# Yukun-Huang/DreamWaltz-G

Measured on AMD Instinct MI355X. Metric: SDS steps/sec @512^2, 100k Gaussians, SD1.5+ControlNet; raster Mpix/s vs HBM roofline, higher is better.
Workload: dtype f32x

## Files before the change

### dreamwaltz-g_amd/csrc/gemm.hip

```cpp
#include "dwg_common.h"
#include "dwg_prof_internal.h"
#include "../../include/dwg_gemm.h"
#include <cstdlib>
#include <type_traits>

#if defined(DWG_GEMM_X_TU)
#include "dwg_xfmt.h"
typedef _Float16 HT;
#define DWG_DTYPE_HALF DWG_DTYPE_F32X
#define DWG_MFMA16(a, b, c) __builtin_amdgcn_mfma_f32_32x32x16_f16(a, b, c, 0, 0, 0)
#define DWG_HALF_NAME "f32x"
#elif defined(DWG_GEMM_F16_TU)
typedef _Float16 HT;
#define DWG_DTYPE_HALF DWG_DTYPE_F16
#define DWG_MFMA16(a, b, c) __builtin_amdgcn_mfma_f32_32x32x16_f16(a, b, c, 0, 0, 0)
#define DWG_HALF_NAME "f16"
#else
typedef __bf16 HT;
#define DWG_DTYPE_HALF DWG_DTYPE_BF16
#define DWG_MFMA16(a, b, c) __builtin_amdgcn_mfma_f32_32x32x16_bf16(a, b, c, 0, 0, 0)
#define DWG_HALF_NAME "bf16"
#endif

namespace {

typedef __attribute__((ext_vector_type(8))) HT bf16x8;
typedef __attribute__((ext_vector_type(16))) float f32x16;

struct ConvP {
    int enabled, Cin, Hin, Win, Hout, Wout, KH, KW, stride, pad_t, pad_l, dil;
    int up;
    int cin1;
    const void* A2;
};

struct GemmP {
    const void* A; const void* B; void* C; const void* bias; const void* residual;
    int M, N, K;
    long long sam, sak, sbn, sbk, ldc, ldr;
    int nb2;
    long long bA1, bA2, bB1, bB2, bC1, bC2, bR1, bR2;
    int act; float alpha;
    int out_bf16, res_bf16, bias_per_row, splitk, accumulate;
    float* ws;
    int bias_row_div;
    long long bias_ld;
    ConvP conv;
};

__device__ __forceinline__ float bf2f(HT x) { return (float)x; }
// ... 249 lines not shown
            float4 r = *reinterpret_cast<const float4*>(reinterpret_cast<const float*>(p.residual) + ri);
            v[0] += r.x; v[1] += r.y; v[2] += r.z; v[3] += r.w;
        }
    }
    const long long ci = coff + (long long)row * p.ldc + col;
    if (p.out_bf16) {
        st_half4(p.C, ci, v);
    } else {
        float4* dst = reinterpret_cast<float4*>(reinterpret_cast<float*>(p.C) + ci);
        float4 o = make_float4(v[0], v[1], v[2], v[3]);
        if (p.accumulate) { float4 c = *dst; o.x += c.x; o.y += c.y; o.z += c.z; o.w += c.w; }
        *dst = o;
    }
}

template <int BN, int BM = 128> struct EpiLds {
    static constexpr int LDC = BN + 4;
    static constexpr int passes(size_t lds_bytes) {
        return lds_bytes >= (size_t)BM * LDC * 4 ? 1 : (lds_bytes >= (size_t)(BM / 2) * LDC * 4 ? 2 : 4);
    }
    static constexpr size_t bytes(int npass) { return (size_t)(BM / npass) * LDC * 4; }
};

template <int BN, int NPASS, int TM, int TN, bool LIGHT, int BM = 128, int NT = 256, typename RowFn>
__device__ __forceinline__ void tile_epilogue_lds(const GemmP& p, f32x16 (&acc)[TM][TN], float* sC, int n0, int wm, int wn, int lane, int tid,
                                                  int ks_id, long long coff, long long roff, RowFn row_of) {
    constexpr int LDC = EpiLds<BN, BM>::LDC, C4 = BN / 4, PR = BM / NPASS;
    constexpr int BPP = BM / 32 / NPASS;
    static_assert(NT % C4 == 0 && (C4 & (C4 - 1)) == 0, "a thread keeps one column group");
    const bool vec_ok = epilogue_vec_ok(p, coff, roff);
    const int lrow = lane & 31, lhalf = (lane >> 5) * 4;
    const bool geglu = p.act == 6;
    const float* bias = reinterpret_cast<const float*>(p.bias);
    const bool fast = vec_ok && !geglu && !p.accumulate && !p.bias_per_row && (p.splitk <= 1 || p.ws) &&
                      (!bias || p.bias_row_div > 0 || ((uintptr_t)bias & 15) == 0) &&
                      (!bias || p.bias_row_div <= 0 || (((uintptr_t)bias & 15) == 0 && (p.bias_ld & 3) == 0)) &&
                      (p.splitk <= 1 || ((uintptr_t)p.ws & 15) == 0);
#pragma unroll 1
    for (int q = 0; q < NPASS; q++) {
        __syncthreads();
#pragma unroll
        for (int i = 0; i < TM; i++) {
            const int rb = wm * TM + i;
            if (NPASS > 1 && rb / BPP != q) continue;
            float* dst = sC + ((NPASS > 1 ? rb % BPP : rb) * 32 + lrow) * LDC + wn * 64 + lhalf;
#pragma unroll
            for (int j = 0; j < TN; j++)
#pragma unroll
                for (int r4 = 0; r4 < 4; r4++)
                    *reinterpret_cast<float4*>(dst + j * 32 + 8 * r4) =
                        make_float4(acc[i][j][4 * r4], acc[i][j][4 * r4 + 1], acc[i][j][4 * r4 + 2], acc[i][j][4 * r4 + 3]);
        }
        __syncthreads();
        if (geglu) {
            constexpr int G = C4 / 2, RSTEP = NT / G;
            const int o4 = tid & (G - 1), rl0 = tid / G;
            const int b = o4 >> 3, w = (o4 & 7) * 4;
            const int colp = n0 + b * 64 + w;
            if (colp + 35 < p.N) {
                float bh[4] = {0.f, 0.f, 0.f, 0.f}, bg[4] = {0.f, 0.f, 0.f, 0.f};
                if (bias) {
#pragma unroll
                    for (int e = 0; e < 4; e++) { bh[e] = bias[colp + e]; bg[e] = bias[colp + 32 + e]; }
                }
                const bool vec_store = ((p.ldc | coff) & 3) == 0 && ((uintptr_t)p.C & 7) == 0;
#pragma unroll 2
                for (int rl = rl0; rl < PR; rl += RSTEP) {
                    const int row = row_of(q * PR + rl);
                    if (row < 0) continue;
                    const float4 h = *reinterpret_cast<const float4*>(sC + rl * LDC + b * 64 + w);
                    const float4 g = *reinterpret_cast<const float4*>(sC + rl * LDC + b * 64 + 32 + w);
                    const float hv[4] = {h.x, h.y, h.z, h.w}, gv[4] = {g.x, g.y, g.z, g.w};
                    float v[4];
#pragma unroll
// ... 344 lines not shown
    }
    __device__ __forceinline__ void issue(unsigned char* lds_tile, const ConvP& cv) {
        const int wave = __builtin_amdgcn_readfirstlane(threadIdx.x >> 6);
        const unsigned char* zero = g_zero16;
        const bool second = CAT && ci >= cv.cin1;
        const int cs = CAT ? (second ? cv.Cin - cv.cin1 : cv.cin1) : cv.Cin;
        const long long uoff = (((long long)ky * cv.Win + kx) * cs + (second ? ci - cv.cin1 : ci)) * 2;
        const unsigned int bit = kcur < kend ? (1u << tap) : 0u;
#pragma unroll
        for (int j = 0; j < NJ; j++) {
            const unsigned char* src = (mask[j] & bit) ? ((CAT && second) ? pb2[j] : pb[j]) + uoff : zero;
            unsigned char* dst = lds_tile + ((wave * NJ + j) * 8) * 128;
            __builtin_amdgcn_global_load_lds((const __attribute__((address_space(1))) void*)src,
                                             (__attribute__((address_space(3))) void*)dst, 16, 0, 0);
        }
    }
};

template <int N>
__device__ __forceinline__ void wait_vmcnt() {
    __builtin_amdgcn_s_waitcnt((N & 15) | ((N >> 4) << 14) | (7 << 4) | (15 << 8));
}

template <int BM, int AKIND, int NW = 4> struct ALoaderOf { typedef GldsLoader<BM, false, NW> type; };
template <int BM, int NW> struct ALoaderOf<BM, 1, NW> { typedef GldsLoader<BM, true, NW> type; };
template <int BM, int NW> struct ALoaderOf<BM, 2, NW> { typedef GldsConvFast<BM, NW, false> type; };
template <int BM, int NW> struct ALoaderOf<BM, 3, NW> { typedef GldsConvFast<BM, NW, true> type; };

template <int BM, int BN> struct GldsGeom {
    static constexpr int WN = BN / 64, WM = (BM == 128 && BN == 64) ? 4 : BM / 64, NW = WM * WN, NT = NW * 64, TM = BM / WM / 32, TN = 2;
};

template <int BM, int BN, int AKIND, int S>
__device__ __forceinline__ void gemm_glds_body(const GemmP& p) {
    typedef GldsGeom<BM, BN> Geo;
    constexpr int WN = Geo::WN, WM = Geo::WM, NW = Geo::NW, NT = Geo::NT, TM = Geo::TM, TN = Geo::TN;
    constexpr int ABYTES = BM * 128, BBYTES = BN * 128, STAGE = ABYTES + BBYTES;
    extern __shared__ __attribute__((aligned(16))) unsigned char smem_raw[];
    const int tid = threadIdx.x, lane = tid & 63, wave = tid >> 6;
    const int wm = wave / WN, wn = wave % WN;
    const int gm = (p.M + BM - 1) / BM, ntn = (p.N + BN - 1) / BN;
    const int nwg = gridDim.x;
    int id = blockIdx.x;
    {
        const int q = nwg / 8, r = nwg % 8, xcd = id % 8, loc = id / 8;
        id = (xcd < r ? xcd * (q + 1) : r * (q + 1) + (xcd - r) * q) + loc;
    }
    const int tile = id % (gm * ntn), ks_id = id / (gm * ntn);
    const int m0 = (tile / ntn) * BM, n0 = (tile % ntn) * BN;
    const int z = blockIdx.z, z1 = z / p.nb2, z2 = z - z1 * p.nb2;
    const HT* A = reinterpret_cast<const HT*>(p.A) + z1 * p.bA1 + z2 * p.bA2;
    const HT* B = reinterpret_cast<const HT*>(p.B) + z1 * p.bB1 + z2 * p.bB2;
    int kbeg = 0, kend = p.K;
    if (p.splitk > 1) {
        int per = ((p.K + p.splitk - 1) / p.splitk + 63) / 64 * 64;
        kbeg = ks_id * per; kend = min(p.K, kbeg + per);
    }
    f32x16 acc[TM][TN];
#pragma unroll
    for (int i = 0; i < TM; i++)
#pragma unroll
        for (int j = 0; j < TN; j++)
#pragma unroll
            for (int r = 0; r < 16; r++) acc[i][j][r] = 0.f;
#ifdef DWG_GEMM_X_TU
    f32x16 acx[TM][TN];
#pragma unroll
    for (int i = 0; i < TM; i++)
#pragma unroll
        for (int j = 0; j < TN; j++)
#pragma unroll
            for (int r = 0; r < 16; r++) acx[i][j][r] = 0.f;
#endif
    typename ALoaderOf<BM, AKIND, NW>::type la;
    GldsLoader<BN, false, NW> lb;
    la.init(A, p.sam, p.M, m0, kbeg, kend, p.conv);
    lb.init(B, p.sbn, p.N, n0, kbeg, kend, p.conv);
    const int nk = kend > kbeg ? (kend - kbeg + 63) / 64 : 0;
    constexpr int LPT = (BM + BN) * 128 / (NT * 16);
#pragma unroll
    for (int s = 0; s < S - 1; s++) {
        la.issue(smem_raw + s * STAGE, p.conv); lb.issue(smem_raw + s * STAGE + ABYTES, p.conv);
        la.advance(p.conv); lb.advance(p.conv);
    }
    const int frow = lane & 31, fx = (lane >> 1) & 7, fh = lane >> 5;
#ifdef DWG_GEMM_X_TU
    constexpr int KS = 2;
    struct Frag { bf16x8 ah[TM], al[TM], bh[TN], bl[TN]; };
#else
    constexpr int KS = 4;
    struct Frag { bf16x8 af[TM], bf[TN]; };
#endif
    auto load_frags = [&](int stage, int ks, Frag& f) {
        const unsigned char* ta = smem_raw + stage * STAGE + (wm * TM * 32 + frow) * 128;
        const unsigned char* tb = smem_raw + stage * STAGE + ABYTES + (wn * 64 + frow) * 128;
#ifdef DWG_GEMM_X_TU
        const int offh = (((ks * 4 + fh * 2) ^ fx) << 4), offl = (((ks * 4 + fh * 2 + 1) ^ fx) << 4);
#pragma unroll
        for (int i = 0; i < TM; i++) {
            f.ah[i] = *reinterpret_cast<const bf16x8*>(ta + i * 32 * 128 + offh);
            f.al[i] = *reinterpret_cast<const bf16x8*>(ta + i * 32 * 128 + offl);
        }
#pragma unroll
        for (int j = 0; j < TN; j++) {
            f.bh[j] = *reinterpret_cast<const bf16x8*>(tb + j * 32 * 128 + offh);
            f.bl[j] = *reinterpret_cast<const bf16x8*>(tb + j * 32 * 128 + offl);
        }
#else
        const int off = (((ks * 2 + fh) ^ fx) << 4);
#pragma unroll
        for (int i = 0; i < TM; i++) f.af[i] = *reinterpret_cast<const bf16x8*>(ta + i * 32 * 128 + off);
#pragma unroll
        for (int j = 0; j < TN; j++) f.bf[j] = *reinterpret_cast<const bf16x8*>(tb + j * 32 * 128 + off);
#endif
    };
    auto mma = [&](const Frag& f) {
#ifdef DWG_GEMM_X_TU
#pragma unroll
        for (int i = 0; i < TM; i++)
#pragma unroll
            for (int j = 0; j < TN; j++) acc[i][j] = DWG_MFMA16(f.bh[j], f.ah[i], acc[i][j]);
#pragma unroll
        for (int i = 0; i < TM; i++)
#pragma unroll
            for (int j = 0; j < TN; j++) acx[i][j] = DWG_MFMA16(f.bl[j], f.ah[i], acx[i][j]);
#pragma unroll
        for (int i = 0; i < TM; i++)
#pragma unroll
            for (int j = 0; j < TN; j++) acx[i][j] = DWG_MFMA16(f.bh[j], f.al[i], acx[i][j]);
#else
#pragma unroll
        for (int i = 0; i < TM; i++)
#pragma unroll
            for (int j = 0; j < TN; j++) acc[i][j] = DWG_MFMA16(f.bf[j], f.af[i], acc[i][j]);
#endif
    };
    auto wait_tile_and_lds = [&]() {
        constexpr int N = (S - 2) * LPT;
        __builtin_amdgcn_s_waitcnt((N & 15) | ((N >> 4) << 14) | (7 << 4) | (0 << 8));
    };
    Frag F[2];
    int cur = 0, nxt = S - 1;
    if (nk > 0) {
        wait_vmcnt<(S - 2) * LPT>();
        __builtin_amdgcn_s_barrier();
        load_frags(0, 0, F[0]);
        __builtin_amdgcn_s_waitcnt(0xC07F);
    }
#ifdef DWG_GEMM_X_TU
    constexpr int MPS = 3 * TM * TN;
#else
    constexpr int MPS = TM * TN;
#endif
    for (int kt = 0; kt < nk; kt++) {
        const int cnext = cur + 1 == S ? 0 : cur + 1;
#pragma unroll
        for (int ks = 0; ks < KS; ks++) {
            if (ks + 1 < KS) {
                load_frags(cur, ks + 1, F[(ks + 1) & 1]);
            } else {
                wait_tile_and_lds();
                __builtin_amdgcn_s_barrier();
                load_frags(cnext, 0, F[0]);
            }
            __builtin_amdgcn_sched_barrier(0);
            if (ks == 0) {
                la.issue(smem_raw + nxt * STAGE, p.conv); lb.issue(smem_raw + nxt * STAGE + ABYTES, p.conv);
                la.advance(p.conv); lb.advance(p.conv);
            }
            mma(F[ks & 1]);
            if (ks == 0) {
#pragma unroll
                for (int m = 0; m < MPS; m++) {
                    __builtin_amdgcn_sched_group_barrier(0x008, 1, 0);
                    __builtin_amdgcn_sched_group_barrier(0x006, (LPT * 10 + MPS - 1) / MPS, 0);
                    __builtin_amdgcn_sched_group_barrier(0x020, (LPT + MPS - 1) / MPS, 0);
                }
            }
            __builtin_amdgcn_sched_barrier(0);
        }
        __builtin_amdgcn_s_waitcnt(0xC07F);
        cur = cnext; nxt = nxt + 1 == S ? 0 : nxt + 1;
    }
    wait_vmcnt<0>();
#ifdef DWG_GEMM_X_TU
#pragma unroll
    for (int i = 0; i < TM; i++)
#pragma unroll
        for (int j = 0; j < TN; j++)
#pragma unroll
            for (int r = 0; r < 16; r++) acc[i][j][r] = fmaf(acx[i][j][r], DWG_X_LO_INV, acc[i][j][r]);
#endif
    constexpr int NPASS = EpiLds<BN, BM>::passes((size_t)S * STAGE);
    static_assert((size_t)S * STAGE >= EpiLds<BN, BM>::bytes(NPASS), "epilogue staging fits in the operand stages");
    tile_epilogue_lds<BN, NPASS, TM, TN, false, BM, NT>(p, acc, reinterpret_cast<float*>(smem_raw), n0, wm, wn, lane, tid, ks_id, z1 * p.bC1 + z2 * p.bC2,
                                         z1 * p.bR1 + z2 * p.bR2, [&](int rl) { const int r = m0 + rl; return r < p.M ? r : -1; });
}

template <int BN, int AKIND, int S>
__global__ __launch_bounds__(256, 2) void k_gemm_glds(GemmP p) {
    gemm_glds_body<128, BN, AKIND, S>(p);
}

template <int BM, int BN, int AKIND, int S>
__global__ __launch_bounds__(512, 2) void k_gemm_glds8(GemmP p) {
    static_assert(GldsGeom<BM, BN>::NT == 512, "eight waves");
    gemm_glds_body<BM, BN, AKIND, S>(p);
}

static double gemm_flops(const GemmP& p, int batch) {
    double f = 2.0 * p.M * p.N * p.K * batch;
#ifdef DWG_GEMM_X_TU
    f *= 0.5;
#endif
    if (p.conv.enabled && p.conv.dil > 1) f /= (double)(p.conv.dil * p.conv.dil);
    return f;
}

template <int BN, int AKIND>
static void launch_glds(const GemmP& p, int batch, hipStream_t stream, const char* name) {
    constexpr int S = (BN == 64 && AKIND != 1) ? 3 : 2;
    size_t lds = (size_t)S * (128 + BN) * 128;
    static bool attr_set = false;
// ... 5 lines not shown
    static const char* const sym[2][4] = {{"k_gemm_glds<64, 0, 3>", "k_gemm_glds<64, 1, 2>", "k_gemm_glds<64, 2, 3>", "k_gemm_glds<64, 3, 3>"},
                                          {"k_gemm_glds<128, 0, 2>", "k_gemm_glds<128, 1, 2>", "k_gemm_glds<128, 2, 2>", "k_gemm_glds<128, 3, 2>"}};
    DWG_LAUNCH_W(name, sym[BN == 128][AKIND], gemm_flops(p, batch), (k_gemm_glds<BN, AKIND, S>), grid, dim3(256), lds, stream, p);
    launch_splitk_epilogue(p, stream);
}

template <int BM, int BN, int AKIND>
static void launch_glds8(const GemmP& p, int batch, hipStream_t stream, const char* name) {
    constexpr int S = 3;
    const size_t lds = (size_t)S * (BM + BN) * 128;
    static bool attr_set = false;
    if (!attr_set) {
        hipFuncSetAttribute(reinterpret_cast<const void*>(&k_gemm_glds8<BM, BN, AKIND, S>), hipFuncAttributeMaxDynamicSharedMemorySize, (int)lds);
        attr_set = true;
    }
    dim3 grid(((p.M + BM - 1) / BM) * ((p.N + BN - 1) / BN) * (p.splitk > 1 ? p.splitk : 1), 1, batch);
    static const char* const sym[2][4] = {
        {"k_gemm_glds8<256, 128, 0, 3>", "k_gemm_glds8<256, 128, 1, 3>", "k_gemm_glds8<256, 128, 2, 3>", "k_gemm_glds8<256, 128, 3, 3>"},
        {"k_gemm_glds8<128, 256, 0, 3>", "k_gemm_glds8<128, 256, 1, 3>", "k_gemm_glds8<128, 256, 2, 3>", "k_gemm_glds8<128, 256, 3, 3>"}};
    DWG_LAUNCH_W(name, sym[BN == 256][AKIND], gemm_flops(p, batch), (k_gemm_glds8<BM, BN, AKIND, S>), grid, dim3(512), lds, stream, p);
    launch_splitk_epilogue(p, stream);
}

template <bool V> struct BoolC { static constexpr bool value = V; };
template <int BN, int NW> struct Patch2Geom {
    static constexpr int PH = NW == 8 ? 16 : 8, PW = 16, HP = PH + 2, WP = PW + 2, NPIX = HP * WP, BM = PH * PW;
    static constexpr int NPI = (NPIX + 7) / 8;
    static constexpr int PPW = (NPI + NW - 1) / NW;
    static constexpr int WN = BN / 64, WM = NW / WN, TM = BM / WM / 32, TN = 2, NT = NW * 64;
    static constexpr int NJW = BN / (8 * NW);
    static constexpr int PBYTES = NPI * 8 * 128, BBYTES = BN * 128;
};

template <int BN, bool SPLIT, int NW, int NBS>
__global__ __launch_bounds__(NW * 64, 2) void k_conv3x3_patch2(GemmP p) {
    typedef Patch2Geom<BN, NW> G;
    constexpr int PH = G::PH, PW = G::PW, WP = G::WP, NPIX = G::NPIX, NPI = G::NPI, PPW = G::PPW;
    constexpr int WN = G::WN, WM = G::WM, TM = G::TM, TN = G::TN, NT = G::NT, NJW = G::NJW, BM = G::BM;
    constexpr int PBYTES = G::PBYTES, BBYTES = G::BBYTES;
    static_assert(NJW >= 1 && (NJW % 2 == 0 || NJW == 1), "row-block parity");
    extern __shared__ __attribute__((aligned(16))) unsigned char smem_raw[];
    unsigned char* sP = smem_raw;
    unsigned char* sB = smem_raw + 2 * PBYTES;
    const ConvP& cv = p.conv;
    const int tid = threadIdx.x, lane = tid & 63, wave = tid >> 6;
    const int wv = __builtin_amdgcn_readfirstlane(wave);
    const int wm = wave / WN, wn = wave % WN;
// ... 24 lines not shown
            const int py = pi / WP, px = pi - py * WP;
            const int iy = y0 - 1 + py, ix = x0 - 1 + px;
            const bool ok = valid && pi < NPIX && iy >= 0 && iy < cv.Hin && ix >= 0 && ix < cv.Win;
            const HT* src = ok ? X + ((long long)iy * cv.Win + ix) * cv.Cin + (lg0 ^ ((inst & 1) << 2)) * 8 + cc * 64 : zero;
            __builtin_amdgcn_global_load_lds((const __attribute__((address_space(1))) void*)src,
                                             (__attribute__((address_space(3))) void*)(dst + inst * 8 * 128), 16, 0, 0);
        }
    };
    const HT* wrow[NJW];
#pragma unroll
    for (int j = 0; j < NJW; j++) {
        const int r = n0 + (wv * NJW + j) * 8 + sub;
        wrow[j] = r < p.N ? Wt + (long long)r * p.sbn + (lg0 ^ (((wv * NJW + j) & 1) << 2)) * 8 : nullptr;
    }
    auto issue_w = [&](int cc, int tap, bool valid, unsigned char* dst) {
        const long long kofs = (long long)tap * cv.Cin + cc * 64;
#pragma unroll
        for (int j = 0; j < NJW; j++) {
            const HT* src = (valid && wrow[j]) ? wrow[j] + kofs : zero;
            __builtin_amdgcn_global_load_lds((const __attribute__((address_space(1))) void*)src,
                                             (__attribute__((address_space(3))) void*)(dst + (wv * NJW + j) * 8 * 128), 16, 0, 0);
        }
    };
    f32x16 acc[TM][TN];
#pragma unroll
    for (int i = 0; i < TM; i++)
#pragma unroll
        for (int j = 0; j < TN; j++)
#pragma unroll
            for (int r = 0; r < 16; r++) acc[i][j][r] = 0.f;
#ifdef DWG_GEMM_X_TU
    f32x16 acx[TM][TN];
#pragma unroll
    for (int i = 0; i < TM; i++)
#pragma unroll
        for (int j = 0; j < TN; j++)
#pragma unroll
            for (int r = 0; r < 16; r++) acx[i][j][r] = 0.f;
    constexpr int KS = 2, MPS = 3 * TM * TN;
    struct Frag { bf16x8 ah[TM], al[TM], bh[TN], bl[TN]; };
#else
    constexpr int KS = 4, MPS = TM * TN;
    struct Frag { bf16x8 af[TM], bf[TN]; };
#endif
    int pbase[TM];
#pragma unroll
    for (int i = 0; i < TM; i++) {
        const int r = (wm * TM + i) * 32 + (lane & 31);
        pbase[i] = (r / PW) * WP + (r % PW);
    }
    int cc0 = 0, ncc = cv.Cin / 64;
    if constexpr (SPLIT) {
        const int per = (ncc + p.splitk - 1) / p.splitk;
        cc0 = ks_id * per; ncc = min(ncc, cc0 + per);
    }
    const int frow = lane & 31, fx = (lane >> 1) & 7, fh = lane >> 5;
    const int nsteps = max(0, ncc - cc0) * 9;
    auto load_frags = [&](const unsigned char* pa, int toff, const unsigned char* tbs, int ks, Frag& f) {
        const unsigned char* tb = tbs + (wn * 64 + frow) * 128;
#ifdef DWG_GEMM_X_TU
        const int cl = ks * 4 + fh * 2;
#pragma unroll
        for (int i = 0; i < TM; i++) {
            const int pi = pbase[i] + toff, sw = (pi >> 1) & 7;
            f.ah[i] = *reinterpret_cast<const bf16x8*>(pa + pi * 128 + ((cl ^ sw) << 4));
            f.al[i] = *reinterpret_cast<const bf16x8*>(pa + pi * 128 + (((cl + 1) ^ sw) << 4));
        }
#pragma unroll
        for (int j = 0; j < TN; j++) {
            f.bh[j] = *reinterpret_cast<const bf16x8*>(tb + j * 32 * 128 + ((cl ^ fx) << 4));
            f.bl[j] = *reinterpret_cast<const bf16x8*>(tb + j * 32 * 128 + (((cl + 1) ^ fx) << 4));
        }
#else
        const int cl = ks * 2 + fh;
#pragma unroll
        for (int i = 0; i < TM; i++) {
            const int pi = pbase[i] + toff;
            f.af[i] = *reinterpret_cast<const bf16x8*>(pa + pi * 128 + ((cl ^ ((pi >> 1) & 7)) << 4));
        }
#pragma unroll
        for (int j = 0; j < TN; j++) f.bf[j] = *reinterpret_cast<const bf16x8*>(tb + j * 32 * 128 + ((cl ^ fx) << 4));
#endif
    };
    auto mma = [&](const Frag& f) {
#ifdef DWG_GEMM_X_TU
#pragma unroll
        for (int i = 0; i < TM; i++)
#pragma unroll
            for (int j = 0; j < TN; j++) acc[i][j] = DWG_MFMA16(f.bh[j], f.ah[i], acc[i][j]);
#pragma unroll
        for (int i = 0; i < TM; i++)
#pragma unroll
            for (int j = 0; j < TN; j++) acx[i][j] = DWG_MFMA16(f.bl[j], f.ah[i], acx[i][j]);
#pragma unroll
        for (int i = 0; i < TM; i++)
#pragma unroll
            for (int j = 0; j < TN; j++) acx[i][j] = DWG_MFMA16(f.bh[j], f.al[i], acx[i][j]);
#else
#pragma unroll
        for (int i = 0; i < TM; i++)
#pragma unroll
            for (int j = 0; j < TN; j++) acc[i][j] = DWG_MFMA16(f.bf[j], f.af[i], acc[i][j]);
#endif
    };
    issue_patch(cc0, nsteps > 0, sP + (cc0 & 1) * PBYTES);
#pragma unroll
    for (int g = 0; g < NBS - 1; g++) issue_w(cc0 + g / 9, g % 9, g < nsteps, sB + g * BBYTES);
    Frag F[2];
    if (nsteps > 0) {
        wait_vmcnt<(NBS - 2) * NJW>();
        __builtin_amdgcn_s_barrier();
        load_frags(sP + (cc0 & 1) * PBYTES, 0, sB, 0, F[0]);
        __builtin_amdgcn_s_waitcnt(0xC07F);
    }
    int bst = 0;
    auto step = [&](auto is_tap0, int tap, int cc, const unsigned char* pa, const unsigned char* pan) {
        constexpr bool TAP0 = decltype(is_tap0)::value;
        const int ty = tap >= 6 ? 2 : (tap >= 3 ? 1 : 0);
        const int toff = ty * WP + (tap - 3 * ty);
        const int bnext = bst + 1 == NBS ? 0 : bst + 1;
        const int bfill = bst == 0 ? NBS - 1 : bst - 1;
        const unsigned char* tb = sB + bst * BBYTES;
#pragma unroll
        for (int ks = 0; ks < KS; ks++) {
            if (ks + 1 < KS) {
                load_frags(pa, toff, tb, ks + 1, F[(ks + 1) & 1]);
// ... 11 lines not shown
                load_frags(tap == 8 ? pan : pa, nty * WP + (ntap - 3 * nty), sB + bnext * BBYTES, 0, F[0]);
            }
            __builtin_amdgcn_sched_barrier(0);
            if (ks == 0) {
                const int ft = tap + NBS - 1, fcc = cc + (ft >= 9 ? 1 : 0), ftap = ft >= 9 ? ft - 9 : ft;
                issue_w(fcc, ftap, fcc < ncc, sB + bfill * BBYTES);
                if (TAP0) issue_patch(cc + 1, cc + 1 < ncc, const_cast<unsigned char*>(pan));
            }
            mma(F[ks & 1]);
            if (ks == 0) {
                constexpr int NL = NJW + (TAP0 ? PPW : 0);
#pragma unroll
                for (int m = 0; m < MPS; m++) {
                    __builtin_amdgcn_sched_group_barrier(0x008, 1, 0);
                    __builtin_amdgcn_sched_group_barrier(0x006, (NL * 8 + MPS - 1) / MPS, 0);
                    __builtin_amdgcn_sched_group_barrier(0x020, (NL + MPS - 1) / MPS, 0);
                }
            }
            __builtin_amdgcn_sched_barrier(0);
        }
        __builtin_amdgcn_s_waitcnt(0xC07F);
        bst = bnext;
    };
    for (int cc = cc0; cc < ncc; cc++) {
        const unsigned char* pa = sP + (cc & 1) * PBYTES;
        const unsigned char* pan = sP + ((cc + 1) & 1) * PBYTES;
        step(BoolC<true>{}, 0, cc, pa, pan);
#pragma unroll 1
        for (int tap = 1; tap < 9; tap++) step(BoolC<false>{}, tap, cc, pa, pan);
    }
    wait_vmcnt<0>();
    __builtin_amdgcn_s_barrier();
#ifdef DWG_GEMM_X_TU
#pragma unroll
    for (int i = 0; i < TM; i++)
#pragma unroll
        for (int j = 0; j < TN; j++)
#pragma unroll
            for (int r = 0; r < 16; r++) acc[i][j][r] = fmaf(acx[i][j][r], DWG_X_LO_INV, acc[i][j][r]);
#endif
    constexpr int NPASS = EpiLds<BN, BM>::passes((size_t)2 * PBYTES + NBS * BBYTES);
    static_assert((size_t)2 * PBYTES + NBS * BBYTES >= EpiLds<BN, BM>::bytes(NPASS), "epilogue staging fits in the patch / weight buffers");
    tile_epilogue_lds<BN, NPASS, TM, TN, !SPLIT, BM, NT>(p, acc, reinterpret_cast<float*>(smem_raw), n0, wm, wn, lane, tid, ks_id, 0, 0, [&](int rr) {
        const int y = y0 + rr / PW, x = x0 + rr % PW;
        return (y < cv.Hout && x < cv.Wout) ? (img * cv.Hout + y) * cv.Wout + x : -1;
    });
}

template <int BN, int NW, int NBS>
static void launch_conv3x3_patch2(const GemmP& p, hipStream_t stream, const char* name) {
    typedef Patch2Geom<BN, NW> G;
    const size_t lds = (size_t)2 * G::PBYTES + (size_t)NBS * G::BBYTES;
    const ConvP& cv = p.conv;
    const int nimg = p.M / (cv.Hout * cv.Wout);
    const int gm = nimg * ((cv.Hout + G::PH - 1) / G::PH) * ((cv.Wout + G::PW - 1) / G::PW);
    dim3 grid(gm * ((p.N + BN - 1) / BN) * (p.splitk > 1 ? p.splitk : 1));
    static bool attr_set = false;
    if (!attr_set) {
        hipFuncSetAttribute(reinterpret_cast<const void*>(&k_conv3x3_patch2<BN, false, NW, NBS>), hipFuncAttributeMaxDynamicSharedMemorySize, (int)lds);
        hipFuncSetAttribute(reinterpret_cast<const void*>(&k_conv3x3_patch2<BN, true, NW, NBS>), hipFuncAttributeMaxDynamicSharedMemorySize, (int)lds);
        attr_set = true;
    }
    static_assert((NW == 8 && BN == 128 && NBS == 4) || (NW == 4 && BN == 64 && NBS == 4) || (NW == 4 && BN == 128 && NBS == 2), "symbol table below");
    const char* sym = NW == 8 ? (p.splitk > 1 && p.ws ? "k_conv3x3_patch2<128, true, 8, 4>" : "k_conv3x3_patch2<128, false, 8, 4>")
                              : (BN == 64 ? (p.splitk > 1 && p.ws ? "k_conv3x3_patch2<64, true, 4, 4>" : "k_conv3x3_patch2<64, false, 4, 4>")
                                          : (p.splitk > 1 && p.ws ? "k_conv3x3_patch2<128, true, 4, 2>" : "k_conv3x3_patch2<128, false, 4, 2>"));
// ... 367 lines not shown
```

Before: 41.35.

## Use 16x16x32 MFMA with permlane-swapped split operands for f32x GEMM and conv

```diff
diff --git a/dreamwaltz-g_amd/csrc/gemm.hip b/dreamwaltz-g_amd/csrc/gemm.hip
--- a/dreamwaltz-g_amd/csrc/gemm.hip
+++ b/dreamwaltz-g_amd/csrc/gemm.hip
@@ -3,22 +3,27 @@
 #include "../../include/dwg_gemm.h"
 #include <cstdlib>
 #include <type_traits>
+#include <utility>
 
 #if defined(DWG_GEMM_X_TU)
 #include "dwg_xfmt.h"
 typedef _Float16 HT;
 #define DWG_DTYPE_HALF DWG_DTYPE_F32X
 #define DWG_MFMA16(a, b, c) __builtin_amdgcn_mfma_f32_32x32x16_f16(a, b, c, 0, 0, 0)
+#define DWG_MFMA32(a, b, c) __builtin_amdgcn_mfma_f32_16x16x32_f16(a, b, c, 0, 0, 0)
+#define DWG_MFMA_K32 1
 #define DWG_HALF_NAME "f32x"
 #elif defined(DWG_GEMM_F16_TU)
 typedef _Float16 HT;
 #define DWG_DTYPE_HALF DWG_DTYPE_F16
 #define DWG_MFMA16(a, b, c) __builtin_amdgcn_mfma_f32_32x32x16_f16(a, b, c, 0, 0, 0)
+#define DWG_MFMA_K32 0
 #define DWG_HALF_NAME "f16"
 #else
 typedef __bf16 HT;
 #define DWG_DTYPE_HALF DWG_DTYPE_BF16
 #define DWG_MFMA16(a, b, c) __builtin_amdgcn_mfma_f32_32x32x16_bf16(a, b, c, 0, 0, 0)
+#define DWG_MFMA_K32 0
 #define DWG_HALF_NAME "bf16"
 #endif
 
@@ -26,6 +31,7 @@
 
 typedef __attribute__((ext_vector_type(8))) HT bf16x8;
 typedef __attribute__((ext_vector_type(16))) float f32x16;
+typedef __attribute__((ext_vector_type(4))) float f32x4;
 
 struct ConvP {
     int enabled, Cin, Hin, Win, Hout, Wout, KH, KW, stride, pad_t, pad_l, dil;
@@ -321,11 +327,12 @@
     static constexpr size_t bytes(int npass) { return (size_t)(BM / npass) * LDC * 4; }
 };
 
-template <int BN, int NPASS, int TM, int TN, bool LIGHT, int BM = 128, int NT = 256, typename RowFn>
-__device__ __forceinline__ void tile_epilogue_lds(const GemmP& p, f32x16 (&acc)[TM][TN], float* sC, int n0, int wm, int wn, int lane, int tid,
+template <int BN, int NPASS, int TM, int TN, bool LIGHT, int BM = 128, int NT = 256, typename ACC, typename RowFn>
+__device__ __forceinline__ void tile_epilogue_lds(const GemmP& p, ACC (&acc)[TM][TN], float* sC, int n0, int wm, int wn, int lane, int tid,
                                                   int ks_id, long long coff, long long roff, RowFn row_of) {
     constexpr int LDC = EpiLds<BN, BM>::LDC, C4 = BN / 4, PR = BM / NPASS;
-    constexpr int BPP = BM / 32 / NPASS;
+    constexpr int TR = sizeof(ACC) == sizeof(f32x16) ? 32 : 16;
+    constexpr int BPP = BM / TR / NPASS;
     static_assert(NT % C4 == 0 && (C4 & (C4 - 1)) == 0, "a thread keeps one column group");
     const bool vec_ok = epilogue_vec_ok(p, coff, roff);
     const int lrow = lane & 31, lhalf = (lane >> 5) * 4;
@@ -342,13 +349,20 @@
         for (int i = 0; i < TM; i++) {
             const int rb = wm * TM + i;
             if (NPASS > 1 && rb / BPP != q) continue;
-            float* dst = sC + ((NPASS > 1 ? rb % BPP : rb) * 32 + lrow) * LDC + wn * 64 + lhalf;
-#pragma unroll
-            for (int j = 0; j < TN; j++)
-#pragma unroll
-                for (int r4 = 0; r4 < 4; r4++)
-                    *reinterpret_cast<float4*>(dst + j * 32 + 8 * r4) =
-                        make_float4(acc[i][j][4 * r4], acc[i][j][4 * r4 + 1], acc[i][j][4 * r4 + 2], acc[i][j][4 * r4 + 3]);
+            if constexpr (TR == 32) {
+                float* dst = sC + ((NPASS > 1 ? rb % BPP : rb) * 32 + lrow) * LDC + wn * 64 + lhalf;
+#pragma unroll
+                for (int j = 0; j < TN; j++)
+#pragma unroll
+                    for (int r4 = 0; r4 < 4; r4++)
+                        *reinterpret_cast<float4*>(dst + j * 32 + 8 * r4) =
+                            make_float4(acc[i][j][4 * r4], acc[i][j][4 * r4 + 1], acc[i][j][4 * r4 + 2], acc[i][j][4 * r4 + 3]);
+            } else {
+                float* dst = sC + ((NPASS > 1 ? rb % BPP : rb) * 16 + (lane & 15)) * LDC + wn * 64 + (lane >> 4) * 4;
+#pragma unroll
+                for (int j = 0; j < TN; j++)
+                    *reinterpret_cast<float4*>(dst + j * 16) = make_float4(acc[i][j][0], acc[i][j][1], acc[i][j][2], acc[i][j][3]);
+            }
         }
         __syncthreads();
         if (geglu) {
@@ -739,6 +753,33 @@
     __builtin_amdgcn_s_waitcnt((N & 15) | ((N >> 4) << 14) | (7 << 4) | (15 << 8));
 }
 
+template <bool V> struct BoolC { static constexpr bool value = V; };
+
+#if DWG_MFMA_K32
+template <int N>
+__device__ __forceinline__ void wait_lgkmcnt() {
+    __builtin_amdgcn_s_waitcnt(0xC07F | (N << 8));
+}
+template <int OFF>
+__device__ __forceinline__ void lds_read_frag(bf16x8& v, unsigned addr) {
+    asm volatile("ds_read_b128 %0, %1 offset:%2" : "=v"(v) : "v"(addr), "n"(OFF));
+}
+__device__ __forceinline__ void swap_halves(bf16x8& p, bf16x8& q) {
+    typedef __attribute__((ext_vector_type(4))) unsigned u32x4;
+    u32x4 a = __builtin_bit_cast(u32x4, p), b = __builtin_bit_cast(u32x4, q);
+#pragma unroll
+    for (int d = 0; d < 4; d++) {
+        const auto r = __builtin_amdgcn_permlane32_swap(a[d], b[d], false, false);
+        a[d] = r[0]; b[d] = r[1];
+    }
+    p = __builtin_bit_cast(bf16x8, a); q = __builtin_bit_cast(bf16x8, b);
+}
+template <int... I, typename F>
+__device__ __forceinline__ void static_for_impl(std::integer_sequence<int, I...>, F&& f) { (f(std::integral_constant<int, I>{}), ...); }
+template <int N, typename F>
+__device__ __forceinline__ void static_for(F&& f) { static_for_impl(std::make_integer_sequence<int, N>{}, f); }
+#endif
+
 template <int BM, int AKIND, int NW = 4> struct ALoaderOf { typedef GldsLoader<BM, false, NW> type; };
 template <int BM, int NW> struct ALoaderOf<BM, 1, NW> { typedef GldsLoader<BM, true, NW> type; };
 template <int BM, int NW> struct ALoaderOf<BM, 2, NW> { typedef GldsConvFast<BM, NW, false> type; };
@@ -773,6 +814,14 @@
         int per = ((p.K + p.splitk - 1) / p.splitk + 63) / 64 * 64;
         kbeg = ks_id * per; kend = min(p.K, kbeg + per);
     }
+#if DWG_MFMA_K32
+    constexpr int TM16 = 2 * TM, TN16 = 2 * TN;
+    f32x4 acc[TM16][TN16], acx[TM16][TN16];
+#pragma unroll
+    for (int i = 0; i < TM16; i++)
+#pragma unroll
+        for (int j = 0; j < TN16; j++) acc[i][j] = acx[i][j] = f32x4{0.f, 0.f, 0.f, 0.f};
+#else
     f32x16 acc[TM][TN];
 #pragma unroll
     for (int i = 0; i < TM; i++)
@@ -780,14 +829,6 @@
         for (int j = 0; j < TN; j++)
 #pragma unroll
             for (int r = 0; r < 16; r++) acc[i][j][r] = 0.f;
-#ifdef DWG_GEMM_X_TU
-    f32x16 acx[TM][TN];
-#pragma unroll
-    for (int i = 0; i < TM; i++)
-#pragma unroll
-        for (int j = 0; j < TN; j++)
-#pragma unroll
-            for (int r = 0; r < 16; r++) acx[i][j][r] = 0.f;
 #endif
     typename ALoaderOf<BM, AKIND, NW>::type la;
     GldsLoader<BN, false, NW> lb;
@@ -800,57 +841,135 @@
         la.issue(smem_raw + s * STAGE, p.conv); lb.issue(smem_raw + s * STAGE + ABYTES, p.conv);
         la.advance(p.conv); lb.advance(p.conv);
     }
+#if DWG_MFMA_K32
+    const int frow = lane & 15, fx = (lane >> 1) & 7, fq = lane >> 4;
+    const int foff = ((2 * fq) ^ fx) << 4;
+    const unsigned lds0 = (unsigned)(uintptr_t)(__attribute__((address_space(3))) unsigned char*)smem_raw;
+    const unsigned a_hi = lds0 + (wm * TM16 * 16 + frow) * 128 + foff, a_lo = a_hi ^ 16;
+    const unsigned b_hi = lds0 + ABYTES + (wn * 64 + frow) * 128 + foff, b_lo = b_hi ^ 16;
+    struct Frag { bf16x8 h, l; };
+    struct FragB { bf16x8 h, x1, x2; };
+    Frag FA[2];
+    FragB FB[TN16];
+    auto load_a = [&](int stage, auto ic, Frag& f) {
+        constexpr int OFF = decltype(ic)::value * 2048;
+        lds_read_frag<OFF>(f.h, a_hi + stage * STAGE);
+        lds_read_frag<OFF>(f.l, a_lo + stage * STAGE);
+    };
+    auto load_b_hi = [&](int stage) { static_for<TN16>([&](auto jc) { lds_read_frag<decltype(jc)::value * 2048>(FB[decltype(jc)::value].h, b_hi + stage * STAGE); }); };
+    auto load_b_lo = [&](int stage) { static_for<TN16>([&](auto jc) { lds_read_frag<decltype(jc)::value * 2048>(FB[decltype(jc)::value].x1, b_lo + stage * STAGE); }); };
+    auto cross_b = [&]() {
+#pragma unroll
+        for (int j = 0; j < TN16; j++) { FB[j].x2 = FB[j].h; swap_halves(FB[j].x1, FB[j].x2); }
+    };
+    auto mma_hh = [&](int i, const Frag& a) {
+#pragma unroll
+        for (int j = 0; j < TN16; j++) acc[i][j] = DWG_MFMA32(FB[j].h, a.h, acc[i][j]);
+    };
+    auto mma_x1 = [&](int i, const bf16x8& a1) {
+#pragma unroll
+        for (int j = 0; j < TN16; j++) acx[i][j] = DWG_MFMA32(FB[j].x1, a1, acx[i][j]);
+    };
+    auto mma_x2 = [&](int i, const bf16x8& a2) {
+#pragma unroll
+        for (int j = 0; j < TN16; j++) acx[i][j] = DWG_MFMA32(FB[j].x2, a2, acx[i][j]);
+    };
+    auto spread_loads = [&](auto nloads, auto nmfma) {
+        constexpr int L = decltype(nloads)::value, M = decltype(nmfma)::value;
+#pragma unroll
+        for (int m = 0; m < M; m++) {
+            __builtin_amdgcn_sched_group_barrier(0x008, 1, 0);
+            __builtin_amdgcn_sched_group_barrier(0x006, (L * 10 + M - 1) / M, 0);
+            __builtin_amdgcn_sched_group_barrier(0x020, (L + M - 1) / M, 0);
+        }
+    };
+    constexpr int LA = BM / (8 * NW), LB = BN / (8 * NW);
+    int cur = 0, nxt = S - 1;
+    if (nk > 0) {
+        wait_vmcnt<(S - 2) * LPT>();
+        __builtin_amdgcn_s_barrier();
+        load_a(0, std::integral_constant<int, 0>{}, FA[0]);
+        load_b_hi(0);
+        load_b_lo(0);
+    }
+    for (int kt = 0; kt < nk; kt++) {
+        const int cnext = cur + 1 == S ? 0 : cur + 1;
+        static_for<TM16>([&](auto ic) {
+            constexpr int i = decltype(ic)::value;
+            const Frag& a = FA[i & 1];
+            bf16x8 a1, a2;
+            auto cross_a = [&]() { a1 = a.h; a2 = a.l; swap_halves(a1, a2); };
+            if constexpr (i == 0) {
+                load_a(cur, std::integral_constant<int, 1>{}, FA[1]);
+                wait_lgkmcnt<TN16 + 2>();
+                __builtin_amdgcn_sched_barrier(0);
+                la.issue(smem_raw + nxt * STAGE, p.conv); la.advance(p.conv);
+                mma_hh(0, a);
+                spread_loads(std::integral_constant<int, LA>{}, std::integral_constant<int, TN16>{});
+                __builtin_amdgcn_sched_barrier(0);
+                wait_lgkmcnt<2>();
+                __builtin_amdgcn_sched_barrier(0);
+                lb.issue(smem_raw + nxt * STAGE + ABYTES, p.conv); lb.advance(p.conv);
+                cross_b(); cross_a();
+                mma_x1(0, a1); mma_x2(0, a2);
+                spread_loads(std::integral_constant<int, LB>{}, std::integral_constant<int, 2 * TN16>{});
+            } else if constexpr (i < TM16 - 1) {
+                load_a(cur, std::integral_constant<int, i + 1>{}, FA[(i + 1) & 1]);
+                wait_lgkmcnt<2>();
+                __builtin_amdgcn_sched_barrier(0);
+                cross_a();
+                mma_hh(i, a); mma_x1(i, a1); mma_x2(i, a2);
+            } else {
+                constexpr int N = (S - 2) * LPT;
+                __builtin_amdgcn_s_waitcnt((N & 15) | ((N >> 4) << 14) | (7 << 4) | (0 << 8));
+                __builtin_amdgcn_s_barrier();
+                load_a(cnext, std::integral_constant<int, 0>{}, FA[0]);
+                cross_a();
+                __builtin_amdgcn_sched_barrier(0);
+                mma_hh(i, a);
+                __builtin_amdgcn_sched_barrier(0);
+                load_b_hi(cnext);
+                __builtin_amdgcn_sched_barrier(0);
+                mma_x1(i, a1);
+                __builtin_amdgcn_sched_barrier(0);
+                load_b_lo(cnext);
+                __builtin_amdgcn_sched_barrier(0);
+                mma_x2(i, a2);
+            }
+            __builtin_amdgcn_sched_barrier(0);
+        });
+        cur = cnext; nxt = nxt + 1 == S ? 0 : nxt + 1;
+    }
+    __builtin_amdgcn_s_waitcnt(0x0070);
+    __builtin_amdgcn_sched_barrier(0);
+#pragma unroll
+    for (int i = 0; i < TM16; i++)
+#pragma unroll
+        for (int j = 0; j < TN16; j++)
+#pragma unroll
+            for (int r = 0; r < 4; r++) acc[i][j][r] = fmaf(acx[i][j][r], DWG_X_LO_INV, acc[i][j][r]);
+    constexpr int NPASS = EpiLds<BN, BM>::passes((size_t)S * STAGE);
+    static_assert((size_t)S * STAGE >= EpiLds<BN, BM>::bytes(NPASS), "epilogue staging fits in the operand stages");
+    tile_epilogue_lds<BN, NPASS, TM16, TN16, false, BM, NT>(p, acc, reinterpret_cast<float*>(smem_raw), n0, wm, wn, lane, tid, ks_id, z1 * p.bC1 + z2 * p.bC2,
+                                         z1 * p.bR1 + z2 * p.bR2, [&](int rl) { const int r = m0 + rl; return r < p.M ? r : -1; });
+#else
     const int frow = lane & 31, fx = (lane >> 1) & 7, fh = lane >> 5;
-#ifdef DWG_GEMM_X_TU
-    constexpr int KS = 2;
-    struct Frag { bf16x8 ah[TM], al[TM], bh[TN], bl[TN]; };
-#else
     constexpr int KS = 4;
     struct Frag { bf16x8 af[TM], bf[TN]; };
-#endif
     auto load_frags = [&](int stage, int ks, Frag& f) {
         const unsigned char* ta = smem_raw + stage * STAGE + (wm * TM * 32 + frow) * 128;
         const unsigned char* tb = smem_raw + stage * STAGE + ABYTES + (wn * 64 + frow) * 128;
-#ifdef DWG_GEMM_X_TU
-        const int offh = (((ks * 4 + fh * 2) ^ fx) << 4), offl = (((ks * 4 + fh * 2 + 1) ^ fx) << 4);
-#pragma unroll
-        for (int i = 0; i < TM; i++) {
-            f.ah[i] = *reinterpret_cast<const bf16x8*>(ta + i * 32 * 128 + offh);
-            f.al[i] = *reinterpret_cast<const bf16x8*>(ta + i * 32 * 128 + offl);
-        }
-#pragma unroll
-        for (int j = 0; j < TN; j++) {
-            f.bh[j] = *reinterpret_cast<const bf16x8*>(tb + j * 32 * 128 + offh);
-            f.bl[j] = *reinterpret_cast<const bf16x8*>(tb + j * 32 * 128 + offl);
-        }
-#else
         const int off = (((ks * 2 + fh) ^ fx) << 4);
 #pragma unroll
         for (int i = 0; i < TM; i++) f.af[i] = *reinterpret_cast<const bf16x8*>(ta + i * 32 * 128 + off);
 #pragma unroll
         for (int j = 0; j < TN; j++) f.bf[j] = *reinterpret_cast<const bf16x8*>(tb + j * 32 * 128 + off);
-#endif
     };
     auto mma = [&](const Frag& f) {
-#ifdef DWG_GEMM_X_TU
 #pragma unroll
         for (int i = 0; i < TM; i++)
 #pragma unroll
-            for (int j = 0; j < TN; j++) acc[i][j] = DWG_MFMA16(f.bh[j], f.ah[i], acc[i][j]);
-#pragma unroll
-        for (int i = 0; i < TM; i++)
-#pragma unroll
-            for (int j = 0; j < TN; j++) acx[i][j] = DWG_MFMA16(f.bl[j], f.ah[i], acx[i][j]);
-#pragma unroll
-        for (int i = 0; i < TM; i++)
-#pragma unroll
-            for (int j = 0; j < TN; j++) acx[i][j] = DWG_MFMA16(f.bh[j], f.al[i], acx[i][j]);
-#else
-#pragma unroll
-        for (int i = 0; i < TM; i++)
-#pragma unroll
             for (int j = 0; j < TN; j++) acc[i][j] = DWG_MFMA16(f.bf[j], f.af[i], acc[i][j]);
-#endif
     };
     auto wait_tile_and_lds = [&]() {
         constexpr int N = (S - 2) * LPT;
@@ -864,11 +983,7 @@
         load_frags(0, 0, F[0]);
         __builtin_amdgcn_s_waitcnt(0xC07F);
     }
-#ifdef DWG_GEMM_X_TU
-    constexpr int MPS = 3 * TM * TN;
-#else
     constexpr int MPS = TM * TN;
-#endif
     for (int kt = 0; kt < nk; kt++) {
         const int cnext = cur + 1 == S ? 0 : cur + 1;
 #pragma unroll
@@ -900,22 +1015,15 @@
         cur = cnext; nxt = nxt + 1 == S ? 0 : nxt + 1;
     }
     wait_vmcnt<0>();
-#ifdef DWG_GEMM_X_TU
-#pragma unroll
-    for (int i = 0; i < TM; i++)
-#pragma unroll
-        for (int j = 0; j < TN; j++)
-#pragma unroll
-            for (int r = 0; r < 16; r++) acc[i][j][r] = fmaf(acx[i][j][r], DWG_X_LO_INV, acc[i][j][r]);
-#endif
     constexpr int NPASS = EpiLds<BN, BM>::passes((size_t)S * STAGE);
     static_assert((size_t)S * STAGE >= EpiLds<BN, BM>::bytes(NPASS), "epilogue staging fits in the operand stages");
     tile_epilogue_lds<BN, NPASS, TM, TN, false, BM, NT>(p, acc, reinterpret_cast<float*>(smem_raw), n0, wm, wn, lane, tid, ks_id, z1 * p.bC1 + z2 * p.bC2,
                                          z1 * p.bR1 + z2 * p.bR2, [&](int rl) { const int r = m0 + rl; return r < p.M ? r : -1; });
+#endif
 }
 
 template <int BN, int AKIND, int S>
-__global__ __launch_bounds__(256, 2) void k_gemm_glds(GemmP p) {
+__global__ __launch_bounds__(256, (BN == 64 && AKIND != 1) ? 3 : 2) void k_gemm_glds(GemmP p) {
     gemm_glds_body<128, BN, AKIND, S>(p);
 }
 
@@ -967,7 +1075,6 @@
     launch_splitk_epilogue(p, stream);
 }
 
-template <bool V> struct BoolC { static constexpr bool value = V; };
 template <int BN, int NW> struct Patch2Geom {
     static constexpr int PH = NW == 8 ? 16 : 8, PW = 16, HP = PH + 2, WP = PW + 2, NPIX = HP * WP, BM = PH * PW;
     static constexpr int NPI = (NPIX + 7) / 8;
@@ -1038,56 +1145,162 @@
                                              (__attribute__((address_space(3))) void*)(dst + (wv * NJW + j) * 8 * 128), 16, 0, 0);
         }
     };
-    f32x16 acc[TM][TN];
-#pragma unroll
-    for (int i = 0; i < TM; i++)
-#pragma unroll
-        for (int j = 0; j < TN; j++)
-#pragma unroll
-            for (int r = 0; r < 16; r++) acc[i][j][r] = 0.f;
-#ifdef DWG_GEMM_X_TU
-    f32x16 acx[TM][TN];
-#pragma unroll
-    for (int i = 0; i < TM; i++)
-#pragma unroll
-        for (int j = 0; j < TN; j++)
-#pragma unroll
-            for (int r = 0; r < 16; r++) acx[i][j][r] = 0.f;
-    constexpr int KS = 2, MPS = 3 * TM * TN;
-    struct Frag { bf16x8 ah[TM], al[TM], bh[TN], bl[TN]; };
-#else
-    constexpr int KS = 4, MPS = TM * TN;
-    struct Frag { bf16x8 af[TM], bf[TN]; };
-#endif
-    int pbase[TM];
-#pragma unroll
-    for (int i = 0; i < TM; i++) {
-        const int r = (wm * TM + i) * 32 + (lane & 31);
-        pbase[i] = (r / PW) * WP + (r % PW);
-    }
+#if DWG_MFMA_K32
+    static_assert(PW == 16, "a 16-row fragment tile is one pixel row of the tile");
+    constexpr int TM16 = 2 * TM, TN16 = 2 * TN;
+    f32x4 acc[TM16][TN16], acx[TM16][TN16];
+#pragma unroll
+    for (int i = 0; i < TM16; i++)
+#pragma unroll
+        for (int j = 0; j < TN16; j++) acc[i][j] = acx[i][j] = f32x4{0.f, 0.f, 0.f, 0.f};
+    const int frow = lane & 15, fx = (lane >> 1) & 7, fq = lane >> 4;
+    const int fch = 2 * fq;
+    struct Frag { bf16x8 h, l; };
+    const int pbase = wm * TM16 * WP + frow;
     int cc0 = 0, ncc = cv.Cin / 64;
     if constexpr (SPLIT) {
         const int per = (ncc + p.splitk - 1) / p.splitk;
         cc0 = ks_id * per; ncc = min(ncc, cc0 + per);
     }
+    const int nsteps = max(0, ncc - cc0) * 9;
+    const unsigned lds0 = (unsigned)(uintptr_t)(__attribute__((address_space(3))) unsigned char*)smem_raw;
+    auto lds_of = [&](const unsigned char* q) { return lds0 + (unsigned)(q - smem_raw); };
+    auto load_a = [&](unsigned pa, int toff, int i, Frag& f) {
+        const int pi = pbase + i * WP + toff;
+        const unsigned ad = pa + pi * 128 + ((fch ^ ((pi >> 1) & 7)) << 4);
+        lds_read_frag<0>(f.h, ad);
+        lds_read_frag<0>(f.l, ad ^ 16);
+    };
+    const unsigned b_hi = (wn * 64 + frow) * 128 + ((fch ^ fx) << 4), b_lo = b_hi ^ 16;
+    struct FragB { bf16x8 h, x1, x2; };
+    Frag FA[2];
+    FragB FB[TN16];
+    auto load_b_hi = [&](unsigned tbs) { static_for<TN16>([&](auto jc) { lds_read_frag<decltype(jc)::value * 2048>(FB[decltype(jc)::value].h, tbs + b_hi); }); };
+    auto load_b_lo = [&](unsigned tbs) { static_for<TN16>([&](auto jc) { lds_read_frag<decltype(jc)::value * 2048>(FB[decltype(jc)::value].x1, tbs + b_lo); }); };
+    auto cross_b = [&]() {
+#pragma unroll
+        for (int j = 0; j < TN16; j++) { FB[j].x2 = FB[j].h; swap_halves(FB[j].x1, FB[j].x2); }
+    };
+    auto mma_hh = [&](int i, const Frag& a) {
+#pragma unroll
+        for (int j = 0; j < TN16; j++) acc[i][j] = DWG_MFMA32(FB[j].h, a.h, acc[i][j]);
+    };
+    auto mma_x1 = [&](int i, const bf16x8& a1) {
+#pragma unroll
+        for (int j = 0; j < TN16; j++) acx[i][j] = DWG_MFMA32(FB[j].x1, a1, acx[i][j]);
+    };
+    auto mma_x2 = [&](int i, const bf16x8& a2) {
+#pragma unroll
+        for (int j = 0; j < TN16; j++) acx[i][j] = DWG_MFMA32(FB[j].x2, a2, acx[i][j]);
+    };
+    auto spread_loads = [&](auto nloads, auto nmfma) {
+        constexpr int L = decltype(nloads)::value, M = decltype(nmfma)::value;
+#pragma unroll
+        for (int m = 0; m < M; m++) {
+            __builtin_amdgcn_sched_group_barrier(0x008, 1, 0);
+            __builtin_amdgcn_sched_group_barrier(0x006, (L * 8 + M - 1) / M, 0);
+            __builtin_amdgcn_sched_group_barrier(0x020, (L + M - 1) / M, 0);
+        }
+    };
+    issue_patch(cc0, nsteps > 0, sP + (cc0 & 1) * PBYTES);
+#pragma unroll
+    for (int g = 0; g < NBS - 1; g++) issue_w(cc0 + g / 9, g % 9, g < nsteps, sB + g * BBYTES);
+    if (nsteps > 0) {
+        wait_vmcnt<(NBS - 2) * NJW>();
+        __builtin_amdgcn_s_barrier();
+        load_a(lds_of(sP + (cc0 & 1) * PBYTES), 0, 0, FA[0]);
+        load_b_hi(lds_of(sB));
+        load_b_lo(lds_of(sB));
+    }
+    int bst = 0;
+    auto step = [&](auto is_tap0, int tap, int cc, const unsigned char* pa_, const unsigned char* pan_) {
+        constexpr bool TAP0 = decltype(is_tap0)::value;
+        const unsigned pa = lds_of(pa_), pan = lds_of(pan_);
+        const int ty = tap >= 6 ? 2 : (tap >= 3 ? 1 : 0);
+        const int toff = ty * WP + (tap - 3 * ty);
+        const int bnext = bst + 1 == NBS ? 0 : bst + 1;
+        const int bfill = bst == 0 ? NBS - 1 : bst - 1;
+        const unsigned tbn = lds_of(sB + bnext * BBYTES);
+        const int ntap = tap == 8 ? 0 : tap + 1;
+        const int nty = ntap >= 6 ? 2 : (ntap >= 3 ? 1 : 0);
+        const int ntoff = nty * WP + (ntap - 3 * nty);
+        static_for<TM16>([&](auto ic) {
+            constexpr int i = decltype(ic)::value;
+            const Frag& a = FA[i & 1];
+            bf16x8 a1, a2;
+            auto cross_a = [&]() { a1 = a.h; a2 = a.l; swap_halves(a1, a2); };
+            if constexpr (i == 0) {
+                load_a(pa, toff, 1, FA[1]);
+                wait_lgkmcnt<TN16 + 2>();
+                __builtin_amdgcn_sched_barrier(0);
+                const int ft = tap + NBS - 1, fcc = cc + (ft >= 9 ? 1 : 0), ftap = ft >= 9 ? ft - 9 : ft;
+                issue_w(fcc, ftap, fcc < ncc, sB + bfill * BBYTES);
+                mma_hh(0, a);
+                spread_loads(std::integral_constant<int, NJW>{}, std::integral_constant<int, TN16>{});
+                __builtin_amdgcn_sched_barrier(0);
+                wait_lgkmcnt<2>();
+                __builtin_amdgcn_sched_barrier(0);
+                if (TAP0) issue_patch(cc + 1, cc + 1 < ncc, const_cast<unsigned char*>(pan_));
+                cross_b(); cross_a();
+                mma_x1(0, a1); mma_x2(0, a2);
+                if (TAP0) spread_loads(std::integral_constant<int, PPW>{}, std::integral_constant<int, 2 * TN16>{});
+            } else if constexpr (i < TM16 - 1) {
+                load_a(pa, toff, i + 1, FA[(i + 1) & 1]);
+                wait_lgkmcnt<2>();
+                __builtin_amdgcn_sched_barrier(0);
+                cross_a();
+                mma_hh(i, a); mma_x1(i, a1); mma_x2(i, a2);
+            } else {
+                if (TAP0 || tap <= NBS - 2) {
+                    constexpr int N = (NBS - 2) * NJW + PPW;
+                    __builtin_amdgcn_s_waitcnt((N & 15) | ((N >> 4) << 14) | (7 << 4) | (0 << 8));
+                } else {
+                    constexpr int N = (NBS - 2) * NJW;
+                    __builtin_amdgcn_s_waitcnt((N & 15) | ((N >> 4) << 14) | (7 << 4) | (0 << 8));
+                }
+                __builtin_amdgcn_s_barrier();
+                load_a(tap == 8 ? pan : pa, ntoff, 0, FA[0]);
+                cross_a();
+                __builtin_amdgcn_sched_barrier(0);
+                mma_hh(i, a);
+                __builtin_amdgcn_sched_barrier(0);
+                load_b_hi(tbn);
+                __builtin_amdgcn_sched_barrier(0);
+                mma_x1(i, a1);
+                __builtin_amdgcn_sched_barrier(0);
+                load_b_lo(tbn);
+                __builtin_amdgcn_sched_barrier(0);
+                mma_x2(i, a2);
+            }
+            __builtin_amdgcn_sched_barrier(0);
+        });
+        bst = bnext;
+    };
+#else
+    f32x16 acc[TM][TN];
+#pragma unroll
+    for (int i = 0; i < TM; i++)
+#pragma unroll
+        for (int j = 0; j < TN; j++)
+#pragma unroll
+            for (int r = 0; r < 16; r++) acc[i][j][r] = 0.f;
+    constexpr int KS = 4, MPS = TM * TN;
+    struct Frag { bf16x8 af[TM], bf[TN]; };
+    int pbase[TM];
+#pragma unroll
+    for (int i = 0; i < TM; i++) {
+        const int r = (wm * TM + i) * 32 + (lane & 31);
+        pbase[i] = (r / PW) * WP + (r % PW);
+    }
+    int cc0 = 0, ncc = cv.Cin / 64;
+    if constexpr (SPLIT) {
+        const int per = (ncc + p.splitk - 1) / p.splitk;
+        cc0 = ks_id * per; ncc = min(ncc, cc0 + per);
+    }
     const int frow = lane & 31, fx = (lane >> 1) & 7, fh = lane >> 5;
     const int nsteps = max(0, ncc - cc0) * 9;
     auto load_frags = [&](const unsigned char* pa, int toff, const unsigned char* tbs, int ks, Frag& f) {
         const unsigned char* tb = tbs + (wn * 64 + frow) * 128;
-#ifdef DWG_GEMM_X_TU
-        const int cl = ks * 4 + fh * 2;
-#pragma unroll
-        for (int i = 0; i < TM; i++) {
-            const int pi = pbase[i] + toff, sw = (pi >> 1) & 7;
-            f.ah[i] = *reinterpret_cast<const bf16x8*>(pa + pi * 128 + ((cl ^ sw) << 4));
-            f.al[i] = *reinterpret_cast<const bf16x8*>(pa + pi * 128 + (((cl + 1) ^ sw) << 4));
-        }
-#pragma unroll
-        for (int j = 0; j < TN; j++) {
-            f.bh[j] = *reinterpret_cast<const bf16x8*>(tb + j * 32 * 128 + ((cl ^ fx) << 4));
-            f.bl[j] = *reinterpret_cast<const bf16x8*>(tb + j * 32 * 128 + (((cl + 1) ^ fx) << 4));
-        }
-#else
         const int cl = ks * 2 + fh;
 #pragma unroll
         for (int i = 0; i < TM; i++) {
@@ -1096,28 +1309,12 @@
         }
 #pragma unroll
         for (int j = 0; j < TN; j++) f.bf[j] = *reinterpret_cast<const bf16x8*>(tb + j * 32 * 128 + ((cl ^ fx) << 4));
-#endif
     };
     auto mma = [&](const Frag& f) {
-#ifdef DWG_GEMM_X_TU
 #pragma unroll
         for (int i = 0; i < TM; i++)
 #pragma unroll
-            for (int j = 0; j < TN; j++) acc[i][j] = DWG_MFMA16(f.bh[j], f.ah[i], acc[i][j]);
-#pragma unroll
-        for (int i = 0; i < TM; i++)
-#pragma unroll
-            for (int j = 0; j < TN; j++) acx[i][j] = DWG_MFMA16(f.bl[j], f.ah[i], acx[i][j]);
-#pragma unroll
-        for (int i = 0; i < TM; i++)
-#pragma unroll
-            for (int j = 0; j < TN; j++) acx[i][j] = DWG_MFMA16(f.bh[j], f.al[i], acx[i][j]);
-#else
-#pragma unroll
-        for (int i = 0; i < TM; i++)
-#pragma unroll
             for (int j = 0; j < TN; j++) acc[i][j] = DWG_MFMA16(f.bf[j], f.af[i], acc[i][j]);
-#endif
     };
     issue_patch(cc0, nsteps > 0, sP + (cc0 & 1) * PBYTES);
 #pragma unroll
@@ -1175,6 +1372,7 @@
         __builtin_amdgcn_s_waitcnt(0xC07F);
         bst = bnext;
     };
+#endif
     for (int cc = cc0; cc < ncc; cc++) {
         const unsigned char* pa = sP + (cc & 1) * PBYTES;
         const unsigned char* pan = sP + ((cc + 1) & 1) * PBYTES;
@@ -1182,19 +1380,22 @@
 #pragma unroll 1
         for (int tap = 1; tap < 9; tap++) step(BoolC<false>{}, tap, cc, pa, pan);
     }
-    wait_vmcnt<0>();
+    __builtin_amdgcn_s_waitcnt(0x0070);
     __builtin_amdgcn_s_barrier();
-#ifdef DWG_GEMM_X_TU
-#pragma unroll
-    for (int i = 0; i < TM; i++)
-#pragma unroll
-        for (int j = 0; j < TN; j++)
-#pragma unroll
-            for (int r = 0; r < 16; r++) acc[i][j][r] = fmaf(acx[i][j][r], DWG_X_LO_INV, acc[i][j][r]);
+#if DWG_MFMA_K32
+    constexpr int ETM = TM16, ETN = TN16;
+#pragma unroll
+    for (int i = 0; i < ETM; i++)
+#pragma unroll
+        for (int j = 0; j < ETN; j++)
+#pragma unroll
+            for (int r = 0; r < 4; r++) acc[i][j][r] = fmaf(acx[i][j][r], DWG_X_LO_INV, acc[i][j][r]);
+#else
+    constexpr int ETM = TM, ETN = TN;
 #endif
     constexpr int NPASS = EpiLds<BN, BM>::passes((size_t)2 * PBYTES + NBS * BBYTES);
     static_assert((size_t)2 * PBYTES + NBS * BBYTES >= EpiLds<BN, BM>::bytes(NPASS), "epilogue staging fits in the patch / weight buffers");
-    tile_epilogue_lds<BN, NPASS, TM, TN, !SPLIT, BM, NT>(p, acc, reinterpret_cast<float*>(smem_raw), n0, wm, wn, lane, tid, ks_id, 0, 0, [&](int rr) {
+    tile_epilogue_lds<BN, NPASS, ETM, ETN, !SPLIT, BM, NT>(p, acc, reinterpret_cast<float*>(smem_raw), n0, wm, wn, lane, tid, ks_id, 0, 0, [&](int rr) {
         const int y = y0 + rr / PW, x = x0 + rr % PW;
         return (y < cv.Hout && x < cv.Wout) ? (img * cv.Hout + y) * cv.Wout + x : -1;
     });
```

New measurement: 39.94. -3.4%, worse.
